# 1fni/cuda-spmv-benchmark

Measured on AMD Instinct MI355X. Metric: cg_iterations_per_second, higher is better.
Workload: dtype f64; 1 GPU; CG on the 20000x20000 5-point stencil (400000000 unknowns, 1999920000 nnz), b=1, x0=0, tol 1e-6; grid=20000, unknowns=400000000, nnz=1999920000, partition=1 row slab(s), transport=single rank (no communicator), converged=True

## Files before the change

### cuda-spmv-benchmark_amd/csrc/cg_slab.hip

```cpp
#include <math.h>
#include <stdlib.h>
#include <string.h>

#include <algorithm>
#include <atomic>
#include <chrono>
#include <limits>
#include <mutex>
#include <thread>
#include <vector>

#include "comm.hpp"
#include "device_runtime.hpp"
#include "multi_rhs.hpp"
#include "solve_common.hpp"
#include "stencil_geometry.hpp"
#include "trace_ranges.hpp"
#include "watchdog.hpp"

using namespace spmv_amd;

namespace spmv_amd {
std::vector<double>& last_cg_history();
}
// ... 13 lines not shown
    double* x0_alloc = nullptr;
    double* vec_arena = nullptr;
    double* planes_alloc = nullptr;
    size_t planes_doubles = 0, planes_s_offset = 0;
    SymPlanes planes;
    bool planes_on = false;
    unsigned char* tile_classes = nullptr;
    size_t tile_class_count = 0;
    long long tiles_uniform = 0, tiles_total = 0;
    double quintuple[5] = {0.0, 0.0, 0.0, 0.0, 0.0};
    bool stream_everywhere = false;
    unsigned char *block_map_whole = nullptr, *block_map_interior = nullptr;
    int *slow_list_whole = nullptr, *slow_list_interior = nullptr;
    int slow_count_whole = 0, slow_count_interior = 0;
    int fused_direction = 1;
    bool x0_known_zero = false;
    bool zero_start = true;
#ifdef SPMV_AMD_LAB
    int zero_start_parts = 7;
    bool zero_start_part(int bit) const { return zero_start && (zero_start_parts & bit) != 0; }
#else
    bool zero_start_part(int) const { return zero_start; }
#endif
    bool spmv_with_dot = false;
    const SymPlanes* sym() const { return planes_on ? &planes : nullptr; }
    std::vector<double> placement;
    std::vector<double> tile_runs;
    double setup_ms[5] = {0.0, 0.0, 0.0, 0.0, 0.0};
    bool setup_trials = true;
    double* p_alloc = nullptr;
// ... 69 lines not shown
    s->op = op;
    s->fused = fused_spmv_of(op);
    s->fused_dot = s->fused.partials > 0;
    s->fuse_init_residual = s->fused_dot && s->fused.can_init;
    s->variant_name = s->fused_dot ? "operator/fused-launch" : "operator/run_device+dot";
    if (s->fused.partials > s->partials_cap) {
        device_release(s->partials_spmv);
        s->partials_cap = s->fused.partials;
        s->partials_spmv = device_alloc<double>((size_t)s->partials_cap);
        HIP_CHECK(hipMemset(s->partials_spmv, 0, (size_t)s->partials_cap * sizeof(double)));
    }
}

void place_coefficients(SpmvAmdCgSlab* s);
void tune_tile_runs(SpmvAmdCgSlab* s);

SymPlanes plane_view(const SpmvAmdCgSlab* s, const double* base) {
    SymPlanes v;
    v.ce = base;
    v.s = base + s->planes_s_offset;
    v.cls = s->stream_everywhere ? nullptr : s->tile_classes;
    v.w = s->quintuple[0], v.c = s->quintuple[1], v.e = s->quintuple[2], v.n = s->quintuple[3], v.s5 = s->quintuple[4];
    return v;
}

bool may_take_planes(const SpmvAmdCgSlab* s) {
    const int n = s->grid;
    return s->op == nullptr && n >= 2 && n >= s->shape.knobs.rowlds_min_grid && s->n_local > 0 && s->n_local % n == 0 &&
           s->row_offset % n == 0;
}
// ... 305 lines not shown
    s->A.view.values = s->A.values;
    if (planes) s->planes = plane_view(s, s->planes_alloc);
    for (double* a : s->ring_alloc) HIP_CHECK(hipMemsetAsync(a, 0, s->slot_doubles * sizeof(double), q));
    HIP_CHECK(hipStreamSynchronize(q));
    s->placement = {0.0, (double)tried, before, moved ? after : before};
}

void tune_tile_runs(SpmvAmdCgSlab* s) {
    if (s->op != nullptr || s->ring.size() < 2) return;
    const size_t nl = (size_t)s->n_local;
    hipStream_t q = s->compute;
    double* x = s->ring[1];
    launch_fill(x, nl, 1.0, q);
    HIP_CHECK(hipMemsetAsync(&s->d_s->converged, 0, sizeof(int), q));
    double rec[4] = {0, 0, 0, 0};
    const int run = tune_rowlds_xcd_run(s->A.view, s->shape, x, s->Ap, s->fused_dot ? s->partials_spmv : nullptr, q, rec, s->sym(),
                                        s->plan_whole.block_map);
    HIP_CHECK(hipMemsetAsync(s->ring_alloc[1], 0, s->slot_doubles * sizeof(double), q));
    HIP_CHECK(hipStreamSynchronize(q));
    if (run <= 0) return;
    s->shape.knobs.rowlds_group = run;
    const int lo = s->has_prev ? s->halo : 0, hi = s->n_local - (s->has_next ? s->halo : 0);
    const auto plan = [&](int a, int b) { return plan_stencil5(s->A.view, a, b > a ? b : a, Stencil5Variant::Auto, s->shape); };
    s->plan_whole = plan(0, s->n_local);
    s->plan_interior = plan(lo, hi);
    s->plan_head = plan(0, lo);
    s->plan_tail = plan(hi, s->n_local);
    attach_block_maps(s);
    s->tile_runs.assign(rec, rec + 4);
}

double halo_wait_limit_s(const SpmvAmdCgSlab* s) {
// ... 890 lines not shown
    WatchdogScope guard("gathering the solution on rank 0", s->comm->rank, -1, report_slab_state, s);
    s->comm->gather_to_root(s->x, s->n_local, x_full, counts.data(), displs.data());
    return 0;
}

extern "C" int spmv_amd_cg_slab_history(SpmvAmdCgSlab* s, double* out, int cap) {
    return copy_history(s->history, out, cap);
}

extern "C" int spmv_amd_cg_slab_spmv(SpmvAmdCgSlab* s, const double* x_full, double* y_local) {
    upload(s->p, x_full + s->row_offset, (size_t)s->n_local);
    if (s->has_prev && s->row_offset >= s->halo)
        upload(s->p - s->halo, x_full + s->row_offset - s->halo, (size_t)s->halo);
    if (s->has_next && s->row_offset + s->n_local + s->halo <= s->n)
        upload(s->p + s->n_local, x_full + s->row_offset + s->n_local, (size_t)s->halo);
    slab_spmv(s, s->spmv_with_dot, false, nullptr);
    HIP_CHECK(hipStreamSynchronize(s->compute));
    HIP_CHECK(hipGetLastError());
    download(y_local, s->Ap, (size_t)s->n_local);
    return 0;
}

extern "C" void spmv_amd_cg_slab_info(const SpmvAmdCgSlab* s, int* row_offset, int* n_local,
                                      int* local_nnz) {
    if (row_offset) *row_offset = s->row_offset;
    if (n_local) *n_local = s->n_local;
    if (local_nnz) *local_nnz = (int)s->A.view.nnz_local;
}

extern "C" const char* spmv_amd_cg_slab_variant(const SpmvAmdCgSlab* s) { return s->variant_name; }

// ... 34 lines not shown
    if (strcmp(name, "late_bulk") == 0) s->late_bulk = value != 0, s->late_predict = value == 2;
    else if (strcmp(name, "lead_rows") == 0) s->lead_rows = value < 512 ? 512 : (size_t)value / 512 * 512;
    else if (strcmp(name, "run_ahead") == 0) s->run_ahead = value != 0, s->guess_far_always = value == 2;
    else if (strcmp(name, "no_overlap") == 0) s->no_overlap = value != 0 || s->comm->pipeline_verdict < 0;
    else if (strcmp(name, "stop_at") == 0) s->stop_at = value > 0 ? (int)value : 0;
    else if (strcmp(name, "spmv_event_stride") == 0) s->spmv_event_stride = (int)value;
    else if (strcmp(name, "csr_coefficients") == 0) s->planes_on = value == 0 && s->planes_alloc != nullptr;
    else if (strcmp(name, "stream_coefficients") == 0) {
        s->stream_everywhere = value != 0;
        if (s->planes_alloc != nullptr) s->planes = plane_view(s, s->planes_alloc);
    }
    else if (strcmp(name, "block_rows") == 0) {
        if (value != 0 && value != 4 && value != 8) return -1;
        s->shape.knobs.rowlds_block_rows = (int)value;
        for (Stencil5Plan* p : {&s->plan_whole, &s->plan_interior, &s->plan_head, &s->plan_tail})
            if (p->variant == Stencil5Variant::RowLds) p->block_rows = (int)value;
        build_block_maps(s);
    }
    else if (strcmp(name, "fused_direction") == 0) {
        if (value < 0 || value > 2) return -1;
        s->fused_direction = (int)value;
    }
    else if (strcmp(name, "zero_start_parts") == 0) s->zero_start_parts = (int)value & 7;
    else if (strcmp(name, "zero_start") == 0) s->zero_start = value != 0;
    else if (strcmp(name, "spmv_with_dot") == 0) s->spmv_with_dot = value != 0;
    else return -1;
    return 0;
}

extern "C" long long spmv_amd_cg_slab_block_map(const SpmvAmdCgSlab* s, int which, unsigned char* out, long long cap) {
    const Stencil5Plan& p = which == 0 ? s->plan_whole : s->plan_interior;
    if (p.block_map == nullptr) return 0;
// ... 23 lines not shown
    if (s->ring.size() < 2 || s->comm->exchanges_halos() || !direction_spmv_available(s, false)) return -1;
    const size_t nl = (size_t)s->n_local;
    const int iteration = 3;
    CgScalars sc;
    memset(&sc, 0, sizeof sc);
    sc.beta = beta;
    sc.iterations = iteration;
    sc.converged = converged != 0 ? 1 : 0;
    sc.pAp = std::numeric_limits<double>::quiet_NaN();
    HIP_CHECK(hipMemcpy(s->d_s, &sc, sizeof sc, hipMemcpyHostToDevice));
    upload(s->r, r, nl);
    upload(s->ring[0], p_in, nl);
    HIP_CHECK(hipMemsetAsync(s->ring[1], 0xFF, nl * sizeof(double), s->compute));
    HIP_CHECK(hipMemsetAsync(s->Ap, 0xFF, nl * sizeof(double), s->compute));
    HIP_CHECK(hipMemsetAsync(s->partials_spmv, 0xFF, (size_t)s->plan_whole.partials * sizeof(double), s->compute));
    s->shape.reverse = false;
    s->reduce_mailbox = nullptr;
    const int used = slab_direction_spmv(s, s->ring[0], s->ring[1], iteration_matches != 0 ? iteration : iteration + 1);
    HIP_CHECK(hipStreamSynchronize(s->compute));
    HIP_CHECK(hipGetLastError());
    download(p_out, s->ring[1], nl);
    download(Ap, s->Ap, nl);
    if (partials != nullptr && cap > 0) download(partials, s->partials_spmv, (size_t)std::min(used, cap));
    HIP_CHECK(hipMemcpy(&sc, s->d_s, sizeof sc, hipMemcpyDeviceToHost));
    *pAp = sc.pAp;
    s->p = s->ring[0];
    return used;
}

extern "C" int spmv_amd_cg_slab_initial_stage(SpmvAmdCgSlab* s, double* r0, double* r_vec, double* partials, int cap, int* count, double* rr) {
    const CGConfigMultiGPU any = {1, 0.0, 0, 0};
    const LoopShape L = loop_shape(s, &any);
    const int form = (L.zero_start ? 1 : 0) | (L.r0_in_ring ? 2 : 0);
// ... 264 lines not shown
```

### cuda-spmv-benchmark_amd/csrc/device_runtime.hip

```cpp
#include "device_runtime.hpp"

#include <stdlib.h>

#include <vector>

#include "stencil_geometry.hpp"

namespace spmv_amd {

namespace {
int env_int(const char* name, int fallback) {
    const char* v = getenv(name);
    return (v && *v) ? atoi(v) : fallback;
}

}

int placement_candidates() {
    const int k = env_int("SPMV_AMD_PLACEMENT_CANDIDATES", 3);
    return k < 1 ? 1 : (k > 16 ? 16 : k);
}
int placement_fail_after() {
#ifdef SPMV_AMD_LAB
    return env_int("SPMV_AMD_PLACEMENT_FAIL_AFTER", 0);
#else
    return 0;
#endif
}

LaunchShape current_launch_shape() {
    LaunchShape shape;
    shape.knobs.rowlds_min_grid = env_int("SPMV_AMD_ROWLDS_MIN_GRID", shape.knobs.rowlds_min_grid);
    shape.knobs.rowlds_group = env_int("SPMV_AMD_ROWLDS_GROUP", shape.knobs.rowlds_group);
    if (shape.knobs.rowlds_group < 0 || shape.knobs.rowlds_group > 64) shape.knobs.rowlds_group = 0;
    const int block_rows = env_int("SPMV_AMD_ROWLDS_BLOCK_ROWS", shape.knobs.rowlds_block_rows);
    if (block_rows == 0 || block_rows == 4 || block_rows == 8) shape.knobs.rowlds_block_rows = block_rows;
    shape.knobs.stencil7_rowlds_min_grid = env_int("SPMV_AMD_STENCIL7_ROWLDS_MIN_GRID", shape.knobs.stencil7_rowlds_min_grid);
    return shape;
}

int tune_rowlds_xcd_run(const SlabCsr& m, const LaunchShape& shape, const double* x, double* y, double* d_partials, hipStream_t stream,
                        double* record, const SymPlanes* planes, const unsigned char* block_map) {
    if (shape.knobs.rowlds_group > 0 || m.n_local < (16 << 20)) return 0;
    LaunchShape trial = shape;
    const Stencil5Plan base = plan_stencil5(m, 0, m.n_local, Stencil5Variant::Auto, trial);
    if (base.variant != Stencil5Variant::RowLds) return 0;
    const int rule = base.xcd_run;
    int cand[6] = {rule, rule - 1, rule + 1, rule - 2, rule + 2, 4};
    EventTimer timer;
    double best_ms = 0.0, rule_ms = 0.0;
    int best = rule;
    for (int k = 0; k < 6; ++k) {
        const int g = cand[k];
        bool seen = g < 1 || g > 64;
        for (int j = 0; j < k; ++j) seen = seen || cand[j] == g;
        if (seen) continue;
        trial.knobs.rowlds_group = g;
        Stencil5Plan p = plan_stencil5(m, 0, m.n_local, Stencil5Variant::RowLds, trial);
        p.block_map = block_map;
        float ms[3];
        for (int i = 0; i < 4; ++i) {
            timer.begin(stream);
            (void)launch_stencil5_spmv(m, p, x, y, 1.0, d_partials, nullptr, false, stream, nullptr, planes);
            timer.end(stream);
            const float t = timer.elapsed_ms();
            if (i > 0) ms[i - 1] = t;
        }
        const double med = ms[0] < ms[1] ? (ms[1] < ms[2] ? ms[1] : (ms[0] < ms[2] ? ms[2] : ms[0])) : (ms[0] < ms[2] ? ms[0] : (ms[1] < ms[2] ? ms[2] : ms[1]));
        if (g == rule) rule_ms = med;
        if (best_ms == 0.0 || med < best_ms) best_ms = med, best = g;
    }
    HIP_CHECK(hipGetLastError());
    if (best_ms > 0.995 * rule_ms) best = rule, best_ms = rule_ms;
    if (record) record[0] = rule, record[1] = best, record[2] = rule_ms, record[3] = best_ms;
    return best;
}

void DeviceCsr::allocate(size_t n_local, size_t local_nnz) {
// ... 115 lines not shown
```

### cuda-spmv-benchmark_amd/csrc/device_runtime.hpp

```cpp
#pragma once

#include <hip/hip_runtime.h>

#include "kernels.hpp"
#include "spmv_amd.h"

namespace spmv_amd {

LaunchShape current_launch_shape();

template <class T>
inline T* device_try_alloc(size_t count) {
    void* p = nullptr;
    if (hipMalloc(&p, (count ? count : 1) * sizeof(T)) != hipSuccess) {
        (void)hipGetLastError();
        return nullptr;
    }
    return static_cast<T*>(p);
}

template <class T>
inline T* device_alloc(size_t count) {
    void* p = nullptr;
    HIP_CHECK(hipMalloc(&p, (count ? count : 1) * sizeof(T)));
// ... 52 lines not shown
        cand[n] = c;
        cost[n] = cost_ms(c);
    }
    int best = 0;
    for (int k = 1; k < n; ++k)
        if (cost[k] < cost[best]) best = k;
    for (int k = 0; k < spacers; ++k) HIP_CHECK(hipFree(spacer[k]));
    for (int k = 0; k < n; ++k)
        if (k != best && (k > 0 || release_first)) device_release(cand[k]);
    if (tried) *tried = n;
    if (gain) *gain = cost[best] > 0.0 ? cost[0] / cost[best] : 1.0;
    return cand[best];
}

int tune_rowlds_xcd_run(const SlabCsr& m, const LaunchShape& shape, const double* x, double* y, double* d_partials, hipStream_t stream,
                        double* record = nullptr, const SymPlanes* planes = nullptr, const unsigned char* block_map = nullptr);

struct EventTimer {
    hipEvent_t start = nullptr, stop = nullptr;
    EventTimer() {
        HIP_CHECK(hipEventCreate(&start));
        HIP_CHECK(hipEventCreate(&stop));
    }
    ~EventTimer() {
        (void)hipEventDestroy(start);
        (void)hipEventDestroy(stop);
    }
    void begin(hipStream_t s) { HIP_CHECK(hipEventRecord(start, s)); }
    void end(hipStream_t s) { HIP_CHECK(hipEventRecord(stop, s)); }
    float elapsed_ms() {
        HIP_CHECK(hipEventSynchronize(stop));
// ... 57 lines not shown
```

### cuda-spmv-benchmark_amd/csrc/kernels.hpp

```cpp
#pragma once

#include <hip/hip_runtime.h>
#include <stddef.h>

struct PeerMailbox;

namespace spmv_amd {

struct SlabCsr {
    const int* row_ptr = nullptr;
    const int* col_idx = nullptr;
    const double* values = nullptr;
    int n_local = 0;
    int row_offset = 0;
    long long nnz_local = 0;
    int max_row_nnz = 0;
    long long nnz_base = 0;
    int n_global = 0;
    int grid_size = -1;
    bool verified_stencil = false;
    int halo_before = 0;
    int halo_after = 0;
};

struct Tunables {
    int rowlds_min_grid = 512;
    int rowlds_group = 0;
    int rowlds_block_rows = 4;
    int stencil7_rowlds_min_grid = 64;
};

inline int xcd_run_group(int n, int block_columns, int small_grid_group) {
    if (n < 8000) return small_grid_group;
    const int g = (n + 1100 + 8 * block_columns - 1) / (8 * block_columns);
    return g < 1 ? 1 : (g > 64 ? 64 : g);
}

struct LaunchShape {
    Tunables knobs;
    bool reverse = false;
};

void launch_generate_stencil5_csr(int n, int row_offset, int n_local, long long nnz_base,
                                  double center, double off, int* row_ptr, int* col_idx,
                                  double* values, hipStream_t stream);
void launch_verify_stencil5_csr(const SlabCsr& m, int* d_mismatch, hipStream_t stream);

enum class Stencil5Variant { Auto, RowDirect, RowGeneric, RowLds };
struct Stencil5Plan {
    Stencil5Variant variant = Stencil5Variant::RowGeneric;
    int first_row = 0, last_row = 0;
    int gi_lo = 0, gi_hi = 0;
    int row_blocks = 0;
    int xcd_run = 0;
    int block_rows = 0;
    const unsigned char* block_map = nullptr;
    int partials = 0;
    const char* name = "";
};
Stencil5Plan plan_stencil5(const SlabCsr& m, int first_row, int last_row, Stencil5Variant variant,
                           const LaunchShape& shape);
int rowlds_xcd_run_rule(int n);
struct ResidualOut {
    const double* b;
    double* r;
    double* p;
};
struct SymPlanes {
    const double* ce = nullptr;
    const double* s = nullptr;
    const unsigned char* cls = nullptr;
    double w = 0.0, c = 0.0, e = 0.0, n = 0.0, s5 = 0.0;
};
void launch_fill_sym_planes(const SlabCsr& m, double* ce, double* s, hipStream_t stream);
void launch_classify_tiles(const SlabCsr& m, const double quintuple[5], unsigned char* cls, unsigned long long* d_uniform, hipStream_t stream);
struct ChebStep {
    const double* r = nullptr;
    const double* dinv = nullptr;
    double* d = nullptr;
    double* z_out = nullptr;
    double g = 0.0, h = 0.0;
    int last = 0;
    int* work_count = nullptr;
};
int rowlds_col_tiles(int n);
int rowlds_block_tiles(const Stencil5Plan& plan);
void launch_block_map(const unsigned char* cls, const Stencil5Plan& plan, unsigned char* out, hipStream_t stream);
void launch_verify_sym_planes(const SlabCsr& m, const SymPlanes& planes, int* d_mismatch, hipStream_t stream);

int launch_stencil5_spmv(const SlabCsr& m, const Stencil5Plan& plan, const double* x, double* y, double alpha,
                         double* d_dot_partials, const int* d_skip_flag, bool reverse, hipStream_t stream,
                         const ResidualOut* init = nullptr, const SymPlanes* planes = nullptr, bool x_zero = false);
struct CgScalars;
struct DirectionSpmv {
    const CgScalars* s;
    int iteration;
    bool fma_form;
    const double* r;
    const double* p_in;
    double* p_out;
    const int* slow_list;
// ... 151 lines not shown
```

### cuda-spmv-benchmark_amd/csrc/spmv_kernels.hip

```cpp
#include "kernels.hpp"

#include <stdlib.h>

#include <type_traits>

#include "direction_device.hpp"
#include "reduce_device.hpp"
#include "stencil_geometry.hpp"
#include "stencil_row_device.hpp"
#include "stream_device.hpp"

namespace spmv_amd {
namespace {

constexpr int kBlock = 256;
constexpr int kWavesPerBlock = 4;
__device__ __forceinline__ long long logical_block(int group, long long total) {
    const long long b = blockIdx.x;
    if (group <= 1) return b;
    const long long t = xcd_run_tile<long long>(b, group);
    return t < total ? t : -1;
}

__device__ __forceinline__ double x_at(const double* __restrict__ x, long long local_col,
// ... 246 lines not shown
    if (kDot || kInit || kCheb) dot_acc = wave_sum(dot_acc);
    *dot = dot_acc;
    return true;
}

__device__ __forceinline__ int rowlds_tile_class(const SymPlanes& sp, int li, int col_tiles, int col_tile) {
    return sp.cls != nullptr ? (int)sp.cls[li * col_tiles + col_tile] : 0;
}

__device__ __forceinline__ int rowlds_tile_of_block(int b, int run, int total, int reverse) {
    const int tile = xcd_run_tile<int>(b, run);
    if (tile >= total) return -1;
    return reverse ? total - 1 - tile : tile;
}

template <int kMode>
__global__ __launch_bounds__(64) void stencil5_rowlds_kernel(
    SlabCsr m, const double* __restrict__ x, double* __restrict__ y, double alpha, int gi_lo, int row_step,
    int gfirst, int col_tiles, int total_tiles, int run, int reverse, double* __restrict__ dot_partials,
    const int* __restrict__ skip_flag, ResidualOut res, SymPlanes sp, ChebStep step) {
    __shared__ double strip[5 * kLdsTileCols];
    __shared__ double xrow[kLdsTileCols + 2];
    const int skip = skip_flag != nullptr ? __builtin_nontemporal_load(skip_flag) : 0;
    const int tile = rowlds_tile_of_block((int)blockIdx.x, run, total_tiles, reverse);
    if (tile < 0) return;
    const int row_group = tile / col_tiles;
    const int col_tile = tile - row_group * col_tiles;
    const int li = gi_lo + row_group * row_step;
    const int uniform = rowlds_tile_class(sp, li, col_tiles, col_tile);
    double dot = 0.0;
// ... 41 lines not shown
    double* __restrict__ xrow = lds + 5 * kLdsTileCols;
    const ResidualOut none{nullptr, nullptr, nullptr};
    const int held = gi_hi - li0 < block_rows ? gi_hi - li0 : block_rows;
#pragma unroll 1
    for (int r = 0; r < held; ++r) {
        const int li = li0 + r;
        const int uniform = rowlds_tile_class(sp, li, col_tiles, col_tile);
        double dot = 0.0;
        if (!rowlds_tile<1, false, true>(m, x, y, alpha, li, gfirst + li, j0, lane, skip, strip, xrow, none, &dot, sp, uniform)) return false;
        if (lane == 0) dot_partials[(li - gi_lo) * col_tiles + col_tile] = dot;
        wave_lds_sync();
    }
    return true;
}

template <int kRows>
__global__ __launch_bounds__(64) void stencil5_rowlds_block_kernel(
    SlabCsr m, const double* __restrict__ x, double* __restrict__ y, double alpha, int gi_lo, int gi_hi, int gfirst, int col_tiles,
    int total_blocks, int run, int reverse, double* __restrict__ dot_partials, const int* __restrict__ skip_flag,
    const unsigned char* __restrict__ block_map, SymPlanes sp) {
    constexpr int kRowDoubles = kLdsTileCols + 2;
    constexpr int kFastDoubles = kRows * kRowDoubles, kOneRowDoubles = 5 * kLdsTileCols + kRowDoubles;
    __shared__ double lds[kFastDoubles > kOneRowDoubles ? kFastDoubles : kOneRowDoubles];
    const int skip = skip_flag != nullptr ? __builtin_nontemporal_load(skip_flag) : 0;
    const int block = rowlds_tile_of_block((int)blockIdx.x, run, total_blocks, reverse);
    if (block < 0) return;
    const int row_block = block / col_tiles;
    const int col_tile = block - row_block * col_tiles;
    const int li0 = gi_lo + row_block * kRows;
    const int j0 = col_tile * kLdsTileCols, lane = (int)threadIdx.x;
    const int n = m.grid_size;
    const int fast = (int)block_map[block];
    const int row_lo = -(m.halo_before / n), row_hi = (m.n_local + m.halo_after) / n;
    double xv[kRows + 2][2];
    double xo[kRows];
#pragma unroll
    for (int r = 0; r < kRows + 2; ++r) {
        const int li = li0 - 1 + r;
        xv[r][0] = xv[r][1] = 0.0;
        if (li >= row_lo && li < row_hi) {
            const double* __restrict__ xr = x + ((long long)li * n + j0);
            if (j0 + lane < n) xv[r][0] = xr[lane];
            if (j0 + lane + 64 < n) xv[r][1] = xr[lane + 64];
        }
    }
// ... 27 lines not shown
                if (j < n) {
                    const double xc = xv[r + 1][h], xn = xv[r][h], xs = xv[r + 2][h];
                    const double sum = stencil5_row(j, n, sp.w, xw[h], sp.c, xc, sp.e, xe[h], sp.n, xn, sp.s5, xs);
                    dot = fma(xc, sum, dot);
                    __builtin_nontemporal_store(alpha * sum, y + ((long long)li * n + j));
                }
            }
            dot = wave_sum(dot);
            if (lane == 0) dot_partials[(li - gi_lo) * col_tiles + col_tile] = dot;
        }
    } else {
        rowlds_block_slow_rows(m, x, y, alpha, gi_lo, gi_hi, gfirst, col_tiles, li0, kRows, col_tile, j0, lane, skip, lds, dot_partials, sp);
    }
}

template <int kRows>
__global__ __launch_bounds__(64) void stencil5_direction_block_kernel(
    SlabCsr m, const CgScalars* __restrict__ s, int iteration, int fma_form, const double* __restrict__ rvec, const double* __restrict__ p_in,
    double* __restrict__ p_out, double* __restrict__ y, double alpha, int gi_lo, int gi_hi, int col_tiles, int total_blocks, int run, int reverse,
    double* __restrict__ dot_partials, const unsigned char* __restrict__ block_map, SymPlanes sp) {
    constexpr int kRowDoubles = kLdsTileCols + 2;
    __shared__ double lds[kRows * kRowDoubles];
    if (s->iterations != iteration || s->converged != 0) return;
    const double beta = s->beta;
    const int block = rowlds_tile_of_block((int)blockIdx.x, run, total_blocks, reverse);
    if (block < 0) return;
    const int row_block = block / col_tiles;
    const int col_tile = block - row_block * col_tiles;
    const int li0 = gi_lo + row_block * kRows;
    const int j0 = col_tile * kLdsTileCols, lane = (int)threadIdx.x;
    const int n = m.grid_size;
    const int fast = (int)block_map[block];
    const int rows = m.n_local / n;
    const bool in0 = j0 + lane < n, in1 = j0 + lane + 64 < n;
    double rv[kRows + 2][2], pv[kRows + 2][2];
    double ro[kRows], po[kRows];
#pragma unroll
    for (int r = 0; r < kRows + 2; ++r) {
        const int li = li0 - 1 + r;
        rv[r][0] = rv[r][1] = pv[r][0] = pv[r][1] = 0.0;
        if (li >= 0 && li < rows) {
            const double* __restrict__ rr = rvec + ((long long)li * n + j0);
            const double* __restrict__ pr = p_in + ((long long)li * n + j0);
            if (in0) rv[r][0] = rr[lane], pv[r][0] = pr[lane];
            if (in1) rv[r][1] = rr[lane + 64], pv[r][1] = pr[lane + 64];
// ... 587 lines not shown
void launch_classify_tiles(const SlabCsr& m, const double q[5], unsigned char* cls, unsigned long long* d_uniform, hipStream_t stream) {
    const int n = m.grid_size;
    if (m.n_local == 0 || n <= 0 || m.n_local % n != 0) return;
    const int col_tiles = rowlds_col_tiles(n);
    hipLaunchKernelGGL(classify_tiles_kernel, dim3((unsigned)(m.n_local / n) * (unsigned)col_tiles), dim3(64), 0, stream, m, q[0], q[1], q[2], q[3],
                       q[4], col_tiles, cls, d_uniform);
}

int rowlds_xcd_run_rule(int n) {
    if (n < 8000) return 4;
    const int tiles = (n + kLdsTileCols - 1) / kLdsTileCols;
    const int run = (int)(1.05 * tiles / 8.0 + 0.5);
    return run < 1 ? 1 : (run > 64 ? 64 : run);
}

Stencil5Plan plan_stencil5(const SlabCsr& m, int first_row, int last_row, Stencil5Variant variant,
                           const LaunchShape& shape) {
    Stencil5Plan p;
    const Tunables& knobs = shape.knobs;
    const int n = m.grid_size;
    const bool direct_ok = m.verified_stencil && n >= 2 && m.row_offset % n == 0 &&
                           m.n_local % n == 0 && first_row % n == 0 && last_row % n == 0;
    if (variant == Stencil5Variant::Auto)
        variant = !direct_ok ? Stencil5Variant::RowGeneric : n >= knobs.rowlds_min_grid ? Stencil5Variant::RowLds : Stencil5Variant::RowDirect;
    if (variant != Stencil5Variant::RowGeneric && !direct_ok) variant = Stencil5Variant::RowGeneric;
    p.variant = variant;
    if (variant == Stencil5Variant::RowGeneric) {
        p.row_blocks = (int)blocks_for((long long)last_row - first_row);
        p.partials = p.row_blocks * kWavesPerBlock;
        p.name = m.verified_stencil ? "stencil5/row-generic" : "stencil5/row-generic(csr-loop)";
    } else {
        p.gi_lo = first_row / n;
        p.gi_hi = last_row / n;
        if (variant == Stencil5Variant::RowDirect) {
            p.row_blocks = (int)blocks_for(n);
            p.name = "stencil5/row-direct";
        } else {
            p.row_blocks = (n + kLdsTileCols - 1) / kLdsTileCols;
            p.xcd_run = knobs.rowlds_group > 0 ? knobs.rowlds_group : rowlds_xcd_run_rule(n);
            if (p.xcd_run < 1 || p.xcd_run > 64) p.xcd_run = 4;
            p.name = "stencil5/row-lds";
            p.block_rows = knobs.rowlds_block_rows == 4 || knobs.rowlds_block_rows == 8 ? knobs.rowlds_block_rows : 0;
        }
        p.partials = p.row_blocks * (p.gi_hi - p.gi_lo);
    }
    p.first_row = first_row;
    p.last_row = last_row;
    return p;
}

int launch_stencil5_spmv(const SlabCsr& m, const double* x, double* y, double alpha,
                         int first_row, int last_row, double* d_dot_partials,
                         const int* d_skip_flag, Stencil5Variant variant,
                         const LaunchShape& shape, hipStream_t stream) {
    if (last_row <= first_row) return 0;
    return launch_stencil5_spmv(m, plan_stencil5(m, first_row, last_row, variant, shape), x, y, alpha, d_dot_partials,
                                d_skip_flag, shape.reverse, stream);
// ... 11 lines not shown
        hipLaunchKernelGGL(stencil5_rowlds_zero_kernel, grid, dim3(64), 0, stream, m, x, alpha, gi_lo, row_step, gfirst, p.row_blocks, tiles,
                           p.xcd_run, reverse ? 1 : 0, d_dot_partials, res, sp);
        return;
    }
#define SPMV_AMD_LAUNCH_ROWLDS(MODE)                                                                                   \
    hipLaunchKernelGGL((stencil5_rowlds_kernel<MODE>), grid, dim3(64), 0, stream, m, x, y, alpha, gi_lo, row_step, gfirst, \
                       p.row_blocks, tiles, p.xcd_run, reverse ? 1 : 0, d_dot_partials, d_skip_flag, res, sp, cs)
    const ChebStep cs = step ? *step : ChebStep{};
    if (step) SPMV_AMD_LAUNCH_ROWLDS(3);
    else if (init) SPMV_AMD_LAUNCH_ROWLDS(2);
    else if (d_dot_partials) SPMV_AMD_LAUNCH_ROWLDS(1);
    else SPMV_AMD_LAUNCH_ROWLDS(0);
#undef SPMV_AMD_LAUNCH_ROWLDS
}

void launch_rowlds_block(const SlabCsr& m, const Stencil5Plan& p, const double* x, double* y, double alpha, double* d_dot_partials,
                         const int* d_skip_flag, bool reverse, hipStream_t stream, const SymPlanes& sp) {
    const int blocks = rowlds_block_tiles(p);
    const dim3 grid((unsigned)xcd_padded_grid(blocks, p.xcd_run));
    const int gfirst = m.row_offset / m.grid_size;
#define SPMV_AMD_LAUNCH_ROWLDS_BLOCK(ROWS)                                                                                      \
    hipLaunchKernelGGL((stencil5_rowlds_block_kernel<ROWS>), grid, dim3(64), 0, stream, m, x, y, alpha, p.gi_lo, p.gi_hi, gfirst, \
                       p.row_blocks, blocks, p.xcd_run, reverse ? 1 : 0, d_dot_partials, d_skip_flag, p.block_map, sp)
    if (p.block_rows == 4) SPMV_AMD_LAUNCH_ROWLDS_BLOCK(4);
    else SPMV_AMD_LAUNCH_ROWLDS_BLOCK(8);
#undef SPMV_AMD_LAUNCH_ROWLDS_BLOCK
}
}

int rowlds_block_tiles(const Stencil5Plan& p) {
    if (p.variant != Stencil5Variant::RowLds || p.block_rows <= 0 || p.gi_hi <= p.gi_lo) return 0;
    return (p.gi_hi - p.gi_lo + p.block_rows - 1) / p.block_rows * p.row_blocks;
}

void launch_block_map(const unsigned char* cls, const Stencil5Plan& p, unsigned char* out, hipStream_t stream) {
    const int blocks = rowlds_block_tiles(p);
    if (blocks <= 0) return;
    hipLaunchKernelGGL(block_map_kernel, dim3(blocks_for(blocks)), dim3(kBlock), 0, stream, cls, p.row_blocks, p.gi_lo, p.gi_hi, p.block_rows,
                       blocks, out);
}

int launch_stencil5_spmv(const SlabCsr& m, const Stencil5Plan& p, const double* x, double* y, double alpha,
                         double* d_dot_partials, const int* d_skip_flag, bool reverse, hipStream_t stream,
                         const ResidualOut* init, const SymPlanes* planes, bool x_zero) {
    if (p.last_row <= p.first_row) return 0;
    if (init != nullptr && (p.variant != Stencil5Variant::RowLds || d_dot_partials == nullptr)) {
        fprintf(stderr, "[spmv] the fused initial residual exists for the row-lds kernel only\n");
// ... 26 lines not shown
            if (dot) SPMV_AMD_LAUNCH_ROWS(false, true);
            else SPMV_AMD_LAUNCH_ROWS(false, false);
        }
#undef SPMV_AMD_LAUNCH_ROWS
    }
    return dot ? p.partials : 0;
}

int launch_stencil5_direction_spmv(const SlabCsr& m, const Stencil5Plan& p, const DirectionSpmv& d, double* y, double alpha,
                                   double* d_dot_partials, bool reverse, hipStream_t stream, const SymPlanes& sp) {
    const int blocks = rowlds_block_tiles(p);
    if (blocks <= 0 || p.block_map == nullptr || d_dot_partials == nullptr || sp.cls == nullptr || (d.slow_count > 0 && d.slow_list == nullptr)) {
        fprintf(stderr, "[spmv] the direction update inside the SpMV exists for row-lds plans with a block map only\n");
        exit(EXIT_FAILURE);
    }
    const dim3 grid((unsigned)xcd_padded_grid(blocks, p.xcd_run));
    const int gfirst = m.row_offset / m.grid_size;
#define SPMV_AMD_LAUNCH_DIRECTION_BLOCK(ROWS)                                                                                          \
    hipLaunchKernelGGL((stencil5_direction_block_kernel<ROWS>), grid, dim3(64), 0, stream, m, d.s, d.iteration, d.fma_form ? 1 : 0, d.r, \
                       d.p_in, d.p_out, y, alpha, p.gi_lo, p.gi_hi, p.row_blocks, blocks, p.xcd_run, reverse ? 1 : 0, d_dot_partials,    \
                       p.block_map, sp)
    if (p.block_rows == 4) SPMV_AMD_LAUNCH_DIRECTION_BLOCK(4);
    else SPMV_AMD_LAUNCH_DIRECTION_BLOCK(8);
#undef SPMV_AMD_LAUNCH_DIRECTION_BLOCK
    if (d.slow_count > 0)
        hipLaunchKernelGGL(stencil5_block_list_kernel, dim3((unsigned)d.slow_count), dim3(64), 0, stream, m, d.s, d.iteration, d.p_out, y, alpha,
                           p.gi_lo, p.gi_hi, gfirst, p.row_blocks, p.block_rows, d.slow_list, d_dot_partials, sp);
    return p.partials;
}

int launch_stencil5_cheb_step(const SlabCsr& m, const Stencil5Plan& p, const double* z, const ChebStep& step, double* d_dot_partials,
                              const int* d_skip_flag, hipStream_t stream) {
    if (p.variant != Stencil5Variant::RowLds || p.last_row <= p.first_row) return -1;
    launch_rowlds(m, p, z, nullptr, 1.0, p.gi_lo, 1, p.partials, d_dot_partials, d_skip_flag, false, stream, nullptr, nullptr, &step);
    return p.partials;
}

int launch_stencil5_spmv_first_and_last_gridrow(const SlabCsr& m, const Stencil5Plan& head, const Stencil5Plan& tail, const double* x,
                                                double* y, double alpha, double* d_dot_partials, const int* d_skip_flag,
// ... 138 lines not shown
```

Baseline: 231.6 CG iterations/s.

## Stack several row-block waves per workgroup and tune xcd run on fused direction kernel

Adds a block_stack option so the row-lds block and direction-block kernels can run several 64-lane waves per workgroup, each handling a vertically adjacent row block with its own LDS slice. Outside the lab build the stack is forced to 1, so the default kernels keep their old shape. The xcd-run autotuner now times the fused direction+SpMV kernel when that path will be used, so the chosen run length matches the kernel that actually runs in CG. It also adds lab hooks for sweep direction and xcd_run. The tuning change costs a few extra setup launches and scalar uploads, and may pick a different run length.

```diff
diff --git a/cuda-spmv-benchmark_amd/csrc/cg_slab.hip b/cuda-spmv-benchmark_amd/csrc/cg_slab.hip
--- a/cuda-spmv-benchmark_amd/csrc/cg_slab.hip
+++ b/cuda-spmv-benchmark_amd/csrc/cg_slab.hip
@@ -51,6 +51,7 @@
     int *slow_list_whole = nullptr, *slow_list_interior = nullptr;
     int slow_count_whole = 0, slow_count_interior = 0;
     int fused_direction = 1;
+    bool hook_reverse = false;
     bool x0_known_zero = false;
     bool zero_start = true;
 #ifdef SPMV_AMD_LAB
@@ -150,6 +151,7 @@
 
 void place_coefficients(SpmvAmdCgSlab* s);
 void tune_tile_runs(SpmvAmdCgSlab* s);
+bool direction_spmv_available(const SpmvAmdCgSlab* s, bool cap);
 
 SymPlanes plane_view(const SpmvAmdCgSlab* s, const double* base) {
     SymPlanes v;
@@ -485,8 +487,18 @@
     launch_fill(x, nl, 1.0, q);
     HIP_CHECK(hipMemsetAsync(&s->d_s->converged, 0, sizeof(int), q));
     double rec[4] = {0, 0, 0, 0};
+    const bool fused = s->fused_direction != 0 && !s->comm->exchanges_halos() && direction_spmv_available(s, s->fused_direction != 2);
+    const DirectionSpmv d{s->d_s, 1, s->device_form, s->r, s->ring[0], s->ring[1], s->slow_list_whole, s->slow_count_whole};
+    if (fused) {
+        CgScalars sc;
+        memset(&sc, 0, sizeof sc);
+        sc.beta = 0.5, sc.iterations = 1;
+        HIP_CHECK(hipMemcpyAsync(s->d_s, &sc, sizeof sc, hipMemcpyHostToDevice, q));
+        HIP_CHECK(hipStreamSynchronize(q));
+    }
     const int run = tune_rowlds_xcd_run(s->A.view, s->shape, x, s->Ap, s->fused_dot ? s->partials_spmv : nullptr, q, rec, s->sym(),
-                                        s->plan_whole.block_map);
+                                        s->plan_whole.block_map, fused ? &d : nullptr);
+    if (fused) HIP_CHECK(hipMemsetAsync(s->d_s, 0, sizeof(CgScalars), q));
     HIP_CHECK(hipMemsetAsync(s->ring_alloc[1], 0, s->slot_doubles * sizeof(double), q));
     HIP_CHECK(hipStreamSynchronize(q));
     if (run <= 0) return;
@@ -1407,7 +1419,9 @@
         upload(s->p - s->halo, x_full + s->row_offset - s->halo, (size_t)s->halo);
     if (s->has_next && s->row_offset + s->n_local + s->halo <= s->n)
         upload(s->p + s->n_local, x_full + s->row_offset + s->n_local, (size_t)s->halo);
+    s->shape.reverse = s->hook_reverse;
     slab_spmv(s, s->spmv_with_dot, false, nullptr);
+    s->shape.reverse = false;
     HIP_CHECK(hipStreamSynchronize(s->compute));
     HIP_CHECK(hipGetLastError());
     download(y_local, s->Ap, (size_t)s->n_local);
@@ -1472,8 +1486,23 @@
         if (value != 0 && value != 4 && value != 8) return -1;
         s->shape.knobs.rowlds_block_rows = (int)value;
         for (Stencil5Plan* p : {&s->plan_whole, &s->plan_interior, &s->plan_head, &s->plan_tail})
-            if (p->variant == Stencil5Variant::RowLds) p->block_rows = (int)value;
+            if (p->variant == Stencil5Variant::RowLds)
+                p->block_rows = (int)value, p->block_stack = rowlds_block_stack_for((int)value, s->shape.knobs.rowlds_block_stack);
         build_block_maps(s);
+    }
+    else if (strcmp(name, "block_stack") == 0) {
+        if (value != 1 && value != 2 && value != 4 && value != 8) return -1;
+        if (rowlds_block_stack_for(s->shape.knobs.rowlds_block_rows, (int)value) != (int)value) return -1;
+        s->shape.knobs.rowlds_block_stack = (int)value;
+        for (Stencil5Plan* p : {&s->plan_whole, &s->plan_interior, &s->plan_head, &s->plan_tail})
+            if (p->variant == Stencil5Variant::RowLds) p->block_stack = (int)value;
+    }
+    else if (strcmp(name, "sweep_reverse") == 0) s->hook_reverse = value != 0;
+    else if (strcmp(name, "xcd_run") == 0) {
+        if (value < 1 || value > 64) return -1;
+        s->shape.knobs.rowlds_group = (int)value;
+        for (Stencil5Plan* p : {&s->plan_whole, &s->plan_interior, &s->plan_head, &s->plan_tail})
+            if (p->variant == Stencil5Variant::RowLds) p->xcd_run = (int)value;
     }
     else if (strcmp(name, "fused_direction") == 0) {
         if (value < 0 || value > 2) return -1;
@@ -1527,9 +1556,10 @@
     HIP_CHECK(hipMemsetAsync(s->ring[1], 0xFF, nl * sizeof(double), s->compute));
     HIP_CHECK(hipMemsetAsync(s->Ap, 0xFF, nl * sizeof(double), s->compute));
     HIP_CHECK(hipMemsetAsync(s->partials_spmv, 0xFF, (size_t)s->plan_whole.partials * sizeof(double), s->compute));
-    s->shape.reverse = false;
+    s->shape.reverse = s->hook_reverse;
     s->reduce_mailbox = nullptr;
     const int used = slab_direction_spmv(s, s->ring[0], s->ring[1], iteration_matches != 0 ? iteration : iteration + 1);
+    s->shape.reverse = false;
     HIP_CHECK(hipStreamSynchronize(s->compute));
     HIP_CHECK(hipGetLastError());
     download(p_out, s->ring[1], nl);
diff --git a/cuda-spmv-benchmark_amd/csrc/device_runtime.hip b/cuda-spmv-benchmark_amd/csrc/device_runtime.hip
--- a/cuda-spmv-benchmark_amd/csrc/device_runtime.hip
+++ b/cuda-spmv-benchmark_amd/csrc/device_runtime.hip
@@ -35,12 +35,14 @@
     if (shape.knobs.rowlds_group < 0 || shape.knobs.rowlds_group > 64) shape.knobs.rowlds_group = 0;
     const int block_rows = env_int("SPMV_AMD_ROWLDS_BLOCK_ROWS", shape.knobs.rowlds_block_rows);
     if (block_rows == 0 || block_rows == 4 || block_rows == 8) shape.knobs.rowlds_block_rows = block_rows;
+    const int block_stack = env_int("SPMV_AMD_ROWLDS_BLOCK_STACK", shape.knobs.rowlds_block_stack);
+    if (block_stack == 1 || block_stack == 2 || block_stack == 4 || block_stack == 8) shape.knobs.rowlds_block_stack = block_stack;
     shape.knobs.stencil7_rowlds_min_grid = env_int("SPMV_AMD_STENCIL7_ROWLDS_MIN_GRID", shape.knobs.stencil7_rowlds_min_grid);
     return shape;
 }
 
 int tune_rowlds_xcd_run(const SlabCsr& m, const LaunchShape& shape, const double* x, double* y, double* d_partials, hipStream_t stream,
-                        double* record, const SymPlanes* planes, const unsigned char* block_map) {
+                        double* record, const SymPlanes* planes, const unsigned char* block_map, const DirectionSpmv* fused) {
     if (shape.knobs.rowlds_group > 0 || m.n_local < (16 << 20)) return 0;
     LaunchShape trial = shape;
     const Stencil5Plan base = plan_stencil5(m, 0, m.n_local, Stencil5Variant::Auto, trial);
@@ -61,7 +63,8 @@
         float ms[3];
         for (int i = 0; i < 4; ++i) {
             timer.begin(stream);
-            (void)launch_stencil5_spmv(m, p, x, y, 1.0, d_partials, nullptr, false, stream, nullptr, planes);
+            if (fused != nullptr) (void)launch_stencil5_direction_spmv(m, p, *fused, y, 1.0, d_partials, false, stream, *planes);
+            else (void)launch_stencil5_spmv(m, p, x, y, 1.0, d_partials, nullptr, false, stream, nullptr, planes);
             timer.end(stream);
             const float t = timer.elapsed_ms();
             if (i > 0) ms[i - 1] = t;
diff --git a/cuda-spmv-benchmark_amd/csrc/device_runtime.hpp b/cuda-spmv-benchmark_amd/csrc/device_runtime.hpp
--- a/cuda-spmv-benchmark_amd/csrc/device_runtime.hpp
+++ b/cuda-spmv-benchmark_amd/csrc/device_runtime.hpp
@@ -90,7 +90,8 @@
 }
 
 int tune_rowlds_xcd_run(const SlabCsr& m, const LaunchShape& shape, const double* x, double* y, double* d_partials, hipStream_t stream,
-                        double* record = nullptr, const SymPlanes* planes = nullptr, const unsigned char* block_map = nullptr);
+                        double* record = nullptr, const SymPlanes* planes = nullptr, const unsigned char* block_map = nullptr,
+                        const DirectionSpmv* fused = nullptr);
 
 struct EventTimer {
     hipEvent_t start = nullptr, stop = nullptr;
diff --git a/cuda-spmv-benchmark_amd/csrc/kernels.hpp b/cuda-spmv-benchmark_amd/csrc/kernels.hpp
--- a/cuda-spmv-benchmark_amd/csrc/kernels.hpp
+++ b/cuda-spmv-benchmark_amd/csrc/kernels.hpp
@@ -27,6 +27,7 @@
     int rowlds_min_grid = 512;
     int rowlds_group = 0;
     int rowlds_block_rows = 4;
+    int rowlds_block_stack = 1;
     int stencil7_rowlds_min_grid = 64;
 };
 
@@ -55,12 +56,14 @@
     int xcd_run = 0;
     int block_rows = 0;
     const unsigned char* block_map = nullptr;
+    int block_stack = 1;
     int partials = 0;
     const char* name = "";
 };
 Stencil5Plan plan_stencil5(const SlabCsr& m, int first_row, int last_row, Stencil5Variant variant,
                            const LaunchShape& shape);
 int rowlds_xcd_run_rule(int n);
+int rowlds_block_stack_for(int block_rows, int want);
 struct ResidualOut {
     const double* b;
     double* r;
@@ -85,6 +88,7 @@
 };
 int rowlds_col_tiles(int n);
 int rowlds_block_tiles(const Stencil5Plan& plan);
+int rowlds_block_workgroups(const Stencil5Plan& plan);
 void launch_block_map(const unsigned char* cls, const Stencil5Plan& plan, unsigned char* out, hipStream_t stream);
 void launch_verify_sym_planes(const SlabCsr& m, const SymPlanes& planes, int* d_mismatch, hipStream_t stream);
 
diff --git a/cuda-spmv-benchmark_amd/csrc/spmv_kernels.hip b/cuda-spmv-benchmark_amd/csrc/spmv_kernels.hip
--- a/cuda-spmv-benchmark_amd/csrc/spmv_kernels.hip
+++ b/cuda-spmv-benchmark_amd/csrc/spmv_kernels.hip
@@ -284,6 +284,17 @@
     return reverse ? total - 1 - tile : tile;
 }
 
+template <int kRows, int kStack>
+__device__ __forceinline__ int stacked_block_of_wave(int wave, int run, int total_units, int reverse, int gi_lo, int gi_hi, int col_tiles) {
+    const int unit = rowlds_tile_of_block((int)blockIdx.x, run, total_units, reverse);
+    if constexpr (kStack == 1) return unit;
+    if (unit < 0) return -1;
+    const int unit_row = unit / col_tiles;
+    const int row_block = unit_row * kStack + wave;
+    if (row_block >= (gi_hi - gi_lo + kRows - 1) / kRows) return -1;
+    return unit + (row_block - unit_row) * col_tiles;
+}
+
 template <int kMode>
 __global__ __launch_bounds__(64) void stencil5_rowlds_kernel(
     SlabCsr m, const double* __restrict__ x, double* __restrict__ y, double alpha, int gi_lo, int row_step,
@@ -355,21 +366,25 @@
     return true;
 }
 
-template <int kRows>
-__global__ __launch_bounds__(64) void stencil5_rowlds_block_kernel(
+template <int kRows, int kStack>
+__global__ __launch_bounds__(64 * kStack) void stencil5_rowlds_block_kernel(
     SlabCsr m, const double* __restrict__ x, double* __restrict__ y, double alpha, int gi_lo, int gi_hi, int gfirst, int col_tiles,
-    int total_blocks, int run, int reverse, double* __restrict__ dot_partials, const int* __restrict__ skip_flag,
+    int total_units, int run, int reverse, double* __restrict__ dot_partials, const int* __restrict__ skip_flag,
     const unsigned char* __restrict__ block_map, SymPlanes sp) {
     constexpr int kRowDoubles = kLdsTileCols + 2;
     constexpr int kFastDoubles = kRows * kRowDoubles, kOneRowDoubles = 5 * kLdsTileCols + kRowDoubles;
-    __shared__ double lds[kFastDoubles > kOneRowDoubles ? kFastDoubles : kOneRowDoubles];
+    constexpr int kWaveDoubles = kFastDoubles > kOneRowDoubles ? kFastDoubles : kOneRowDoubles;
+    __shared__ double lds_stack[kStack * kWaveDoubles];
+    const int wave = kStack == 1 ? 0 : __builtin_amdgcn_readfirstlane((int)threadIdx.x >> 6);
+    double* lds = lds_stack;
+    if constexpr (kStack > 1) lds += wave * kWaveDoubles;
     const int skip = skip_flag != nullptr ? __builtin_nontemporal_load(skip_flag) : 0;
-    const int block = rowlds_tile_of_block((int)blockIdx.x, run, total_blocks, reverse);
+    const int block = stacked_block_of_wave<kRows, kStack>(wave, run, total_units, reverse, gi_lo, gi_hi, col_tiles);
     if (block < 0) return;
     const int row_block = block / col_tiles;
     const int col_tile = block - row_block * col_tiles;
     const int li0 = gi_lo + row_block * kRows;
-    const int j0 = col_tile * kLdsTileCols, lane = (int)threadIdx.x;
+    const int j0 = col_tile * kLdsTileCols, lane = kStack == 1 ? (int)threadIdx.x : (int)threadIdx.x & 63;
     const int n = m.grid_size;
     const int fast = (int)block_map[block];
     const int row_lo = -(m.halo_before / n), row_hi = (m.n_local + m.halo_after) / n;
@@ -427,21 +442,24 @@
     }
 }
 
-template <int kRows>
-__global__ __launch_bounds__(64) void stencil5_direction_block_kernel(
+template <int kRows, int kStack>
+__global__ __launch_bounds__(64 * kStack) void stencil5_direction_block_kernel(
     SlabCsr m, const CgScalars* __restrict__ s, int iteration, int fma_form, const double* __restrict__ rvec, const double* __restrict__ p_in,
-    double* __restrict__ p_out, double* __restrict__ y, double alpha, int gi_lo, int gi_hi, int col_tiles, int total_blocks, int run, int reverse,
+    double* __restrict__ p_out, double* __restrict__ y, double alpha, int gi_lo, int gi_hi, int col_tiles, int total_units, int run, int reverse,
     double* __restrict__ dot_partials, const unsigned char* __restrict__ block_map, SymPlanes sp) {
     constexpr int kRowDoubles = kLdsTileCols + 2;
-    __shared__ double lds[kRows * kRowDoubles];
+    __shared__ double lds_stack[kStack * kRows * kRowDoubles];
     if (s->iterations != iteration || s->converged != 0) return;
     const double beta = s->beta;
-    const int block = rowlds_tile_of_block((int)blockIdx.x, run, total_blocks, reverse);
+    const int wave = kStack == 1 ? 0 : __builtin_amdgcn_readfirstlane((int)threadIdx.x >> 6);
+    double* lds = lds_stack;
+    if constexpr (kStack > 1) lds += wave * (kRows * kRowDoubles);
+    const int block = stacked_block_of_wave<kRows, kStack>(wave, run, total_units, reverse, gi_lo, gi_hi, col_tiles);
     if (block < 0) return;
     const int row_block = block / col_tiles;
     const int col_tile = block - row_block * col_tiles;
     const int li0 = gi_lo + row_block * kRows;
-    const int j0 = col_tile * kLdsTileCols, lane = (int)threadIdx.x;
+    const int j0 = col_tile * kLdsTileCols, lane = kStack == 1 ? (int)threadIdx.x : (int)threadIdx.x & 63;
     const int n = m.grid_size;
     const int fast = (int)block_map[block];
     const int rows = m.n_local / n;
@@ -1059,6 +1077,16 @@
     return run < 1 ? 1 : (run > 64 ? 64 : run);
 }
 
+int rowlds_block_stack_for(int block_rows, int want) {
+#ifdef SPMV_AMD_LAB
+    if (want != 1 && want != 2 && want != 4 && want != 8) want = Tunables{}.rowlds_block_stack;
+    return block_rows == 8 && want > 4 ? 4 : want;
+#else
+    (void)block_rows, (void)want;
+    return 1;
+#endif
+}
+
 Stencil5Plan plan_stencil5(const SlabCsr& m, int first_row, int last_row, Stencil5Variant variant,
                            const LaunchShape& shape) {
     Stencil5Plan p;
@@ -1086,6 +1114,7 @@
             if (p.xcd_run < 1 || p.xcd_run > 64) p.xcd_run = 4;
             p.name = "stencil5/row-lds";
             p.block_rows = knobs.rowlds_block_rows == 4 || knobs.rowlds_block_rows == 8 ? knobs.rowlds_block_rows : 0;
+            p.block_stack = rowlds_block_stack_for(p.block_rows, knobs.rowlds_block_stack);
         }
         p.partials = p.row_blocks * (p.gi_hi - p.gi_lo);
     }
@@ -1127,16 +1156,37 @@
 #undef SPMV_AMD_LAUNCH_ROWLDS
 }
 
+#ifdef SPMV_AMD_LAB
+#define SPMV_AMD_FOR_STACKED_BLOCK_SHAPE(SHAPE, LAUNCH) \
+    else if (SHAPE == 4 * 16 + 2) LAUNCH(4, 2);         \
+    else if (SHAPE == 4 * 16 + 4) LAUNCH(4, 4);         \
+    else if (SHAPE == 4 * 16 + 8) LAUNCH(4, 8);         \
+    else if (SHAPE == 8 * 16 + 2) LAUNCH(8, 2);         \
+    else if (SHAPE == 8 * 16 + 4) LAUNCH(8, 4);
+#else
+#define SPMV_AMD_FOR_STACKED_BLOCK_SHAPE(SHAPE, LAUNCH)
+#endif
+#define SPMV_AMD_FOR_BLOCK_SHAPE(PLAN, LAUNCH)                                                                                  \
+    do {                                                                                                                        \
+        const int shape_ = (PLAN).block_rows * 16 + (PLAN).block_stack;                                                         \
+        if (shape_ == 4 * 16 + 1) LAUNCH(4, 1);                                                                                 \
+        else if (shape_ == 8 * 16 + 1) LAUNCH(8, 1);                                                                            \
+        SPMV_AMD_FOR_STACKED_BLOCK_SHAPE(shape_, LAUNCH)                                                                        \
+        else {                                                                                                                  \
+            fprintf(stderr, "[spmv] no block kernel for %d-row blocks stacked %d high\n", (PLAN).block_rows, (PLAN).block_stack); \
+            exit(EXIT_FAILURE);                                                                                                 \
+        }                                                                                                                       \
+    } while (0)
+
 void launch_rowlds_block(const SlabCsr& m, const Stencil5Plan& p, const double* x, double* y, double alpha, double* d_dot_partials,
                          const int* d_skip_flag, bool reverse, hipStream_t stream, const SymPlanes& sp) {
-    const int blocks = rowlds_block_tiles(p);
-    const dim3 grid((unsigned)xcd_padded_grid(blocks, p.xcd_run));
+    const int units = rowlds_block_workgroups(p);
+    const dim3 grid((unsigned)xcd_padded_grid(units, p.xcd_run));
     const int gfirst = m.row_offset / m.grid_size;
-#define SPMV_AMD_LAUNCH_ROWLDS_BLOCK(ROWS)                                                                                      \
-    hipLaunchKernelGGL((stencil5_rowlds_block_kernel<ROWS>), grid, dim3(64), 0, stream, m, x, y, alpha, p.gi_lo, p.gi_hi, gfirst, \
-                       p.row_blocks, blocks, p.xcd_run, reverse ? 1 : 0, d_dot_partials, d_skip_flag, p.block_map, sp)
-    if (p.block_rows == 4) SPMV_AMD_LAUNCH_ROWLDS_BLOCK(4);
-    else SPMV_AMD_LAUNCH_ROWLDS_BLOCK(8);
+#define SPMV_AMD_LAUNCH_ROWLDS_BLOCK(ROWS, STACK)                                                                                     \
+    hipLaunchKernelGGL((stencil5_rowlds_block_kernel<ROWS, STACK>), grid, dim3(64 * STACK), 0, stream, m, x, y, alpha, p.gi_lo, p.gi_hi, \
+                       gfirst, p.row_blocks, units, p.xcd_run, reverse ? 1 : 0, d_dot_partials, d_skip_flag, p.block_map, sp)
+    SPMV_AMD_FOR_BLOCK_SHAPE(p, SPMV_AMD_LAUNCH_ROWLDS_BLOCK);
 #undef SPMV_AMD_LAUNCH_ROWLDS_BLOCK
 }
 }
@@ -1144,6 +1194,12 @@
 int rowlds_block_tiles(const Stencil5Plan& p) {
     if (p.variant != Stencil5Variant::RowLds || p.block_rows <= 0 || p.gi_hi <= p.gi_lo) return 0;
     return (p.gi_hi - p.gi_lo + p.block_rows - 1) / p.block_rows * p.row_blocks;
+}
+
+int rowlds_block_workgroups(const Stencil5Plan& p) {
+    if (rowlds_block_tiles(p) <= 0 || p.block_stack < 1) return 0;
+    const int row_blocks = (p.gi_hi - p.gi_lo + p.block_rows - 1) / p.block_rows;
+    return (row_blocks + p.block_stack - 1) / p.block_stack * p.row_blocks;
 }
 
 void launch_block_map(const unsigned char* cls, const Stencil5Plan& p, unsigned char* out, hipStream_t stream) {
@@ -1200,15 +1256,17 @@
         fprintf(stderr, "[spmv] the direction update inside the SpMV exists for row-lds plans with a block map only\n");
         exit(EXIT_FAILURE);
     }
-    const dim3 grid((unsigned)xcd_padded_grid(blocks, p.xcd_run));
+    const int units = rowlds_block_workgroups(p);
+    const dim3 grid((unsigned)xcd_padded_grid(units, p.xcd_run));
     const int gfirst = m.row_offset / m.grid_size;
-#define SPMV_AMD_LAUNCH_DIRECTION_BLOCK(ROWS)                                                                                          \
-    hipLaunchKernelGGL((stencil5_direction_block_kernel<ROWS>), grid, dim3(64), 0, stream, m, d.s, d.iteration, d.fma_form ? 1 : 0, d.r, \
-                       d.p_in, d.p_out, y, alpha, p.gi_lo, p.gi_hi, p.row_blocks, blocks, p.xcd_run, reverse ? 1 : 0, d_dot_partials,    \
-                       p.block_map, sp)
-    if (p.block_rows == 4) SPMV_AMD_LAUNCH_DIRECTION_BLOCK(4);
-    else SPMV_AMD_LAUNCH_DIRECTION_BLOCK(8);
+#define SPMV_AMD_LAUNCH_DIRECTION_BLOCK(ROWS, STACK)                                                                                       \
+    hipLaunchKernelGGL((stencil5_direction_block_kernel<ROWS, STACK>), grid, dim3(64 * STACK), 0, stream, m, d.s, d.iteration,                \
+                       d.fma_form ? 1 : 0, d.r, d.p_in, d.p_out, y, alpha, p.gi_lo, p.gi_hi, p.row_blocks, units, p.xcd_run, reverse ? 1 : 0, \
+                       d_dot_partials, p.block_map, sp)
+    SPMV_AMD_FOR_BLOCK_SHAPE(p, SPMV_AMD_LAUNCH_DIRECTION_BLOCK);
 #undef SPMV_AMD_LAUNCH_DIRECTION_BLOCK
+#undef SPMV_AMD_FOR_BLOCK_SHAPE
+#undef SPMV_AMD_FOR_STACKED_BLOCK_SHAPE
     if (d.slow_count > 0)
         hipLaunchKernelGGL(stencil5_block_list_kernel, dim3((unsigned)d.slow_count), dim3(64), 0, stream, m, d.s, d.iteration, d.p_out, y, alpha,
                            p.gi_lo, p.gi_hi, gfirst, p.row_blocks, p.block_rows, d.slow_list, d_dot_partials, sp);
```

Result: no change. 232.9 CG iterations/s (median of 2 runs) (+0.6%).
